# Zhehui-Huang/quad-swarm-rl

Hardware: AMD Instinct MI355X
Metric: env-steps/s (drones x envs x sim_steps) (higher is better)
Workload: dtype f32

## Files before the change

__graft_entry__.py:

```python
import os
import subprocess
import sys

REPO = os.path.dirname(os.path.abspath(__file__))
if REPO not in sys.path:
    sys.path.insert(0, REPO)


def build():
    from quad_swarm_rl_amd import native
    native.build(force=True, verbose=True)
    assert os.path.exists(native.LIB_PATH)
    from quad_swarm_rl_amd import policy
    policy.build(force=True, verbose=True)
    assert os.path.exists(policy.ENC_LIB_PATH)
    subprocess.check_call(["make", "-C", os.path.join(REPO, "oracle"), "-s", "-B"])
    import quad_swarm_rl_amd
    from quad_swarm_rl_amd import config, env
    import ctypes
    lib = ctypes.CDLL(native.LIB_PATH)
    for sym in native.EXPORTED_SYMBOLS + native.EXCHANGE_SYMBOLS:
        getattr(lib, sym)
    paths = prebuild_spec_cache()
    print(f"build ok: {native.LIB_PATH} + {len(paths)} config-specialised code objects in spec_cache/")
# ... 32 lines not shown
        import test_object_identity_gpu as toi
        for name in toi.POISON_CASES:
            for team in (0, 1):
                kw = dict(thp.CASES[name], num_envs=7, **toi.POISON_OVERRIDES.get(name, {}))
                prec = "f32" if team and kw["num_agents"] > 8 else "f64"
                jobs.append((kw, prec, team))
                jobs += [(kw, prec, team, {"QS_SPEC_EXTRA_FLAGS": f"-DQS_POISON_IDLE={m}"}) for m in (1, 2)]
        for name in toi.SCHED_SINGLE:
            jobs += [(dict(thp.CASES[name], num_envs=7), "f32", 0), (dict(thp.CASES[name], num_envs=7), "f32", 0, {"QS_SPEC_SINGLE_FLAGS": "-mllvm -amdgpu-use-amdgpu-trackers"})]
        for name in ("c2_n8_dw", "c3_n8_obst", "c4_n32_svs"):
            jobs += [(dict(thp.CASES[name], num_envs=7), "f32", 1), (dict(thp.CASES[name], num_envs=7), "f32", 1, {"QS_SPEC_TEAM_FLAGS": ""})]
        for name in toi.RESPONSE_CASES:
            for prec in ("f64", "f32"):
                if prec == "f64" and thp.CASES[name]["num_agents"] > 8:
                    continue
                jobs += [(dict(thp.CASES[name], num_envs=7), prec, 1), (dict(thp.CASES[name], num_envs=7), prec, 1, {"QS_SPEC_EXTRA_FLAGS": "-DQS_SERIAL_PAIR_RESPONSES"})]
        for name in toi.SELECT_CASES:
            jobs += [(dict(thp.CASES[name], num_envs=7), "f32", 0)] + [(dict(thp.CASES[name], num_envs=7), "f32", 0, {"QS_SPEC_EXTRA_FLAGS": f})
                                                                       for f in ("-DQS_EXACT_NBR_SELECT", "-DQS_NBR_TRUNC_BITS=16")]
        for name in toi.STASH_CASES:
            jobs += [(dict(thp.CASES[name], num_envs=7), "f32", 1), (dict(thp.CASES[name], num_envs=7), "f32", 1, {"QS_SPEC_EXTRA_FLAGS": "-DQS_SN_STASH=0"})]
        for name in toi.REDO_CASES:
            jobs += [(dict(thp.CASES[name], num_envs=7), "f32", 1), (dict(thp.CASES[name], num_envs=7), "f32", 1, {"QS_SPEC_EXTRA_FLAGS": "-DQS_REDO_ROWS=0"})]
        import xchg_worker as xw
        jobs += [(dict(xw.KW, num_envs=8, write_rew_info=False), "f32"), (dict(xw.KW, num_envs=4, episode_sums=True), "f32"),
                 (dict(xw.REPLAY_KW, num_envs=8, write_rew_info=False, episode_sums=True), "f32")]
        import test_pilot_gpu as tpg
        jobs.append((dict(tpg.LOOP_KW, num_envs=1024), "f32"))
        import test_replay_gpu as trg
        jobs += trg.spec_jobs()
    except Exception as exc:
        print("spec prebuild: parity cases skipped:", exc)
    finally:
        sys.path.pop(0)
    if with_audit:
        jobs += _audit_jobs()
    return jobs


def _audit_jobs():
    import base64
    import ctypes
    import json
    from quad_swarm_rl_amd import config as qcfg
    path = os.path.join(REPO, "tests", "spec_audit.json")
    if not os.path.exists(path):
# ... 89 lines not shown
```

quad-swarm-rl_amd/csrc/qs_state_rows.h:

```cpp
#pragma once
#include "qs_state_blk.h"
#include "qs_xchg_dev.h"

template <typename real> struct Ptrs {
    StateBlk blk;
    real *pos, *vel, *rot, *omega, *rot_damp, *cmds_damp, *ou, *goal;
    uint32_t *flags;
    uint64_t *pair_mask, *new_pair_mask;
    real *obs, *reward, *rew_info;
    uint8_t *done;
    int32_t *obst_hit_idx;
    uint64_t *unique_col, *obst_new, *room_new;
    int32_t *counters, *tick;
    uint32_t *step_ctr;
    real *obst_pos;
    real *dist_ring, *dist_sums;
    real *ep_stats;
    int32_t *ep_counters;
    real *scen_real;
    int32_t *scen_int;
    uint32_t *error_flag;
    uint64_t *scen_omap;
    int32_t *scenario_id;
    int32_t *ep_scenario;
// ... 68 lines not shown
            for (int k = 0; k < K; ++k) st(src[k], k);
            return;
        }
        constexpr int D = K * (int)sizeof(T) / 4;
        uint32_t w[D];
#pragma unroll
        for (int k = 0; k < K; ++k) {
            if constexpr (sizeof(T) == 8) { const uint64_t u = __builtin_bit_cast(uint64_t, src[k]); w[2 * k] = (uint32_t)u;
                w[2 * k + 1] = (uint32_t)(u >> 32); }
            else w[k] = __builtin_bit_cast(uint32_t, src[k]);
        }
        st_dwords<D>(w, 0);
    }
};
#define QS_BUF_RSRC(p) __builtin_amdgcn_make_buffer_rsrc((void *)(p).blk.base, 0, (p).blk.bytes, 0x00020000)
#define QS_BLK blockIdx.x
#if defined(QS_SPEC_TEAM)
#define QS_LM(p) (QS_SPEC_TEAM == 8)
#else
#define QS_LM(p) ((p).blk.lane_major != 0)
#endif
#define QS_ROW(TYPE, name, rs, p, T, g) const BufRow<TYPE> b_##name = {rs, (uint32_t)(QS_BLK * (p).blk.block_bytes + (p).blk.name), (uint32_t)((QS_LM(p) ? 1 : 64) * sizeof(TYPE)), \
                                                                       (uint32_t)((threadIdx.x & 63) * ((QS_LM(p) ? blkc::name : 1) * sizeof(TYPE))), QS_LM(p)}
#define QS_ROWF(TYPE, name, rs, p, T, g) const BufRow<TYPE> b_##name = {rs, (p).blk.name, (uint32_t)((T) * sizeof(TYPE)), (uint32_t)((g) * sizeof(TYPE)), false}
```

quad-swarm-rl_amd/csrc/qs_step_team.inc:

```
#undef e_state_or_e
#if QS_MULTI
#define e_state_or_e e_state
#else
#define e_state_or_e e
#endif
#ifndef QS_GATED
#define QS_GATED 0
#endif
#ifdef QS_SPEC
#if QS_MULTI && QS_GATED
extern "C" __global__ void __launch_bounds__(64 * QS_TW) qs_spec_gated(QS_KARGS, int QS_EPB_ARG, int ksteps) {
#elif QS_MULTI
extern "C" __global__ void __launch_bounds__(64 * QS_TW) qs_spec_rollout(QS_KARGS, int QS_EPB_ARG, int ksteps) {
#else
extern "C" __global__ void __launch_bounds__(64 * QS_TW) qs_spec_step(QS_KARGS, int QS_EPB_ARG) {
    const int t = 0;
#endif
#else
template <typename real>
#if QS_MULTI && QS_GATED && QS_SCEN_FULL
__global__ void __launch_bounds__(64 * QS_TW) qs_gated_team_full(QS_KARGS, int QS_EPB_ARG, int ksteps) {
#elif QS_MULTI && QS_GATED
__global__ void __launch_bounds__(64 * QS_TW) qs_gated_team(QS_KARGS, int QS_EPB_ARG, int ksteps) {
#elif QS_MULTI && QS_SCEN_FULL
__global__ void __launch_bounds__(64 * QS_TW) qs_rollout_team_full(QS_KARGS, int QS_EPB_ARG, int ksteps) {
#elif QS_MULTI
__global__ void __launch_bounds__(64 * QS_TW) qs_rollout_team(QS_KARGS, int QS_EPB_ARG, int ksteps) {
#elif QS_SCEN_FULL
__global__ void __launch_bounds__(64 * QS_TW) qs_step_team_full(QS_KARGS, int QS_EPB_ARG) {
    const int t = 0;
// ... 35 lines not shown
#endif
#endif
#ifndef QS_REDO_ROWS
#ifdef QS_SPEC
#define QS_REDO_ROWS 1
#else
#define QS_REDO_ROWS 0
#endif
#endif

    QS_POISON_LDS(L.total, 64 * QS_TW);
    const int wv = __builtin_amdgcn_readfirstlane((int)(threadIdx.x >> 6));
    const int tid = threadIdx.x & 63, le = tid / N, i = tid - le * N, e = blockIdx.x * epb + le, base = le * N;
    const bool active = (le < epb) && (e < E);
    const int g = active ? e * N + i : 0, ee = active ? e : 0;
    const uint64_t nmask = (N >= 64) ? ~0ull : ((1ull << N) - 1);
    real *myobs = s_obs + tid * c.obs_dim;
    const __amdgpu_buffer_rsrc_t rs = QS_BUF_RSRC(p);
    QS_ROW(real, pos, rs, p, T, g); QS_ROW(real, vel, rs, p, T, g); QS_ROW(real, rot, rs, p, T, g); QS_ROW(real, omega, rs, p, T, g);
    QS_ROW(real, rot_damp, rs, p, T, g); QS_ROW(real, cmds_damp, rs, p, T, g); QS_ROW(real, ou, rs, p, T, g);
    QS_ROW(real, goal, rs, p, T, g);
    QS_ROW(real, ring, rs, p, T, g); QS_ROW(real, sums, rs, p, T, g); QS_ROW(uint32_t, flags, rs, p, T, g);
    QS_ROW(uint64_t, pair, rs, p, T, g);

    QS_STAMP(0);
    QS_STAMPW(0);
    QS_STAMP_WG(0);
    Drone<real> d;
    real goal[3], act[4], ring[4], sums[3];
    int32_t cnt[QS_CNT_COUNT];
    uint64_t prev_pair = 0;
    int tick_before = 0, svs_period = 0;
#if QS_SCEN_FULL && defined(QS_SPEC_N)
    ScenRegs<real> sreg;
#endif
    uint32_t step_no = 0;
    uint32_t step_raw = 0;
    if (wv <= 1 || (QS_SN_STASH && !QS_MULTI && wv == 2)) step_raw = p.step_ctr[ee];
    if (wv == 0) {
        if (b_pos.wide) {
            b_pos.template ldv<3>(d.pos); b_vel.template ldv<3>(d.vel); b_omega.template ldv<3>(d.omega); b_goal.template ldv<3>(goal);
            b_sums.template ldv<3>(sums);
            b_rot.template ldv<9>(d.rot);
            b_rot_damp.template ldv<4>(d.rot_damp); b_cmds_damp.template ldv<4>(d.cmds_damp); b_ou.template ldv<4>(d.ou);
            b_ring.template ldv<4>(ring);
        } else {
#pragma unroll
            for (int q = 0; q < 3; ++q) { d.pos[q] = b_pos.ld(q); d.vel[q] = b_vel.ld(q); d.omega[q] = b_omega.ld(q);
                goal[q] = b_goal.ld(q); sums[q] = b_sums.ld(q); }
#pragma unroll
            for (int q = 0; q < 9; ++q) d.rot[q] = b_rot.ld(q);
#pragma unroll
            for (int q = 0; q < 4; ++q) { d.rot_damp[q] = b_rot_damp.ld(q); d.cmds_damp[q] = b_cmds_damp.ld(q); d.ou[q] = b_ou.ld(q);
                ring[q] = b_ring.ld(q); }
        }
        d.flags = b_flags.ld();
        prev_pair = b_pair.ld();
        QS_POISON_DRONE(d); QS_POISON_ARR(goal, 3, 16); QS_POISON_ARR(sums, 3, 16); QS_POISON_ARR(ring, 4, 16); QS_POISON_U64(prev_pair);
        tick_before = p.tick[ee];
        svs_period = (c.scenario == QS_SCENARIO_SWARM_VS_SWARM) ? p.scen_int[ee] : 0;
        if (active && i == 0) {
// ... 9 lines not shown
#endif
        asm volatile("" : "+v"(step_raw));
        step_no = step_raw + 1;
    } else if (wv == 1 || (QS_SN_STASH && !QS_MULTI && wv == 2)) {
        step_no = step_raw + 1;
    }
    if (wv == W - 1 && c.use_obstacles && active) {
        for (int k = i; k < M_; k += N) {
            s_obst[(le * 2 + 0) * M_ + k] = p.obst_pos[(size_t)e * M_ + k];
            s_obst[(le * 2 + 1) * M_ + k] = p.obst_pos[(size_t)E * M_ + (size_t)e * M_ + k];
        }
    }
#if QS_SCEN_FULL
    real *s_sr = (real *)(smem + L.off_sr) + le * SR_COUNT;
    int *s_si = (int *)(smem + L.off_si) + le * SI_COUNT;
#endif
    constexpr int WL = 2;
    const bool logw = (wv == WL) && active;
    real rsum[QS_SUM_COUNT];
    if (logw && c.episode_sums) {
#pragma unroll
        for (int q = 0; q < QS_SUM_COUNT; ++q) rsum[q] = p.run_sums[q * T + g];
    }
#if !QS_MULTI
    unsigned long long xq_seq = 0, xq_ack = ~0ull;
    if constexpr (sizeof(real) == 4) {
        if (p.xchg != nullptr) {
            xq_seq = p.xchg->loc->push_seq;
            if (wv == 0 && tid < p.xchg->world) xq_ack = qsx::ld_sys(&p.xchg->mine->ack[tid]);
        }
    }
#endif
    uint64_t out_curr_pair = 0;
    bool nan_any = false;
#if QS_MULTI
    const int g_state = g, e_state = e;
#if QS_GATED
    qsx::Gate *const G = (qsx::Gate *)p.xchg;
    const unsigned long long gseq0 = (unsigned long long)(uintptr_t)actions;
    bool gate_dead = false;
    unsigned long long *s_pre_seq = (unsigned long long *)s_ri;
    unsigned int *s_actpre = (unsigned int *)((char *)s_ri + 16);
    unsigned long long pf_flag = 0, pf_flag_next = 0;
    if (threadIdx.x == 0) *s_pre_seq = 0;
#endif
    for (int t = 0; t < ksteps; ++t) {
    int g = g_state, e = e_state;
// ... 670 lines not shown
        int nenv = E - first_env; nenv = nenv < epb ? nenv : epb;
        const int total = nenv * N * D;
        real *dst = p.obs + (size_t)first_env * N * D;
#if QS_GATED
        {
            if ((total & 3) == 0 && ((((size_t)first_env * N * D) * sizeof(real)) & 15) == 0 && sizeof(real) == 4) {
                const qsx::u32x4_t *src4 = (const qsx::u32x4_t *)s_obs;
                for (int idx = threadIdx.x; idx < total / 4; idx += 64 * W) qsx::st16_sc1((float *)dst + 4 * idx, src4[idx]);
            } else if constexpr (sizeof(real) == 4) {
                for (int idx = threadIdx.x; idx < total; idx += 64 * W) qsx::st4_sc1(dst + idx, __float_as_uint((float)s_obs[idx]));
            } else {
                for (int idx = threadIdx.x; idx < total; idx += 64 * W) qsx::st8_sc1(dst + idx,
                    (unsigned long long)__double_as_longlong((double)s_obs[idx]));
            }
        }
#else
        if ((total & 3) == 0 && ((((size_t)first_env * N * D) * sizeof(real)) & 15) == 0 && sizeof(real) == 4) {
            const qs_f32x4 *src4 = (const qs_f32x4 *)s_obs;
            for (int idx = threadIdx.x; idx < total / 4; idx += 64 * W) obs_st4((float *)dst + 4 * idx, src4[idx]);
        } else {
            for (int idx = threadIdx.x; idx < total; idx += 64 * W) obs_st1<real>(dst + idx, s_obs[idx]);
        }
#endif
#if !QS_MULTI
        if constexpr (sizeof(real) == 4) {
            if (p.xchg != nullptr) {
                const qsx::XchgDev &X = *p.xchg;
                const unsigned long long seq = xq_seq + 1;
                const int slot = (int)(seq & 1);
                if (wv == 0) {
                    bool ok = true;
                    if (tid < X.world && seq > 2 && xq_ack < seq - 2) ok = qsx::poll_ge(&X.mine->ack[tid], seq - 2, X.timeout_ticks);
                    if (__any(!ok) && tid == 0) atomicOr(&X.loc->status, (unsigned int)QS_XCHG_ERR_ACK_TIMEOUT);
                }
                __syncthreads();
                const size_t row0 = (size_t)first_env * N * D, wsz = X.wire == QS_WIRE_BF16 ? 2 : 4;
                const size_t off = X.wire == QS_WIRE_Q8 ? (size_t)slot * (size_t)X.slot_bytes + ((size_t)X.rank * (size_t)(X.n / D) + (size_t)first_env * N) * (size_t)X.q8.row_words * 4
                                                        : (size_t)slot * (size_t)X.slot_bytes + ((size_t)X.rank * (size_t)X.n + row0) * wsz;
                const float *src = (const float *)s_obs;
                const bool vec = ((total & 7) == 0) && ((off & 15) == 0);
#ifndef QS_NO_Q8_FUSED
                if (X.wire == QS_WIRE_Q8) {
                    const int q0 = c.self_dim, q1 = c.self_dim + 6 * K, w16 = (D - 6 * K + 1) >> 1;
                    const float s0 = X.q8.s0, s1 = X.q8.s1, s2 = X.q8.s2, s3 = X.q8.s3, s4 = X.q8.s4, s5 = X.q8.s5;
                    const int rw = w16 + ((6 * K + 3) >> 2), words = nenv * N * rw;
                    unsigned int *s_wire = (unsigned int *)s_ri;
                    if ((off & 15) == 0 && (words & 3) == 0 && words * 4 <= (int)(sizeof(real) * (QS_RI_COUNT + 1) * B)) {
// ... 103 lines not shown
                qsx::st8_sc1(p.room_new + e, out_room); }
        }
        if (wv == 1) {
            if (pf_hold_issue) {
#pragma unroll
                for (int q = 0; q < (int)sizeof(real); ++q) s_actpre[tid * (int)sizeof(real) + q] = pf_hold[q];
            }
            if (tid == 0) *s_pre_seq = pf_hold_issue ? gseq0 + (unsigned long long)t + 2 : 0ull;
            pf_flag = pf_flag_next;
        }
        asm volatile("s_waitcnt vmcnt(0)" ::: "memory");
        QS_TEAM_BARRIER();
        if (threadIdx.x == 0) qsx::st_agent(&G->done_flag[blockIdx.x], gseq0 + (unsigned long long)t + 1);
    }
#else
    if (wv == 0 && active) {
        {
            QS_ROWF(uint64_t, newpair, rs, p, T, g); QS_ROWF(int32_t, ohit, rs, p, T, g); QS_ROWF(real, reward, rs, p, T, g);
            QS_ROWF(uint8_t, done, rs, p, T, g);
            b_newpair.st(out_new_pair);
            if (c.use_obstacles) b_ohit.st(out_obst_idx);
            b_reward.st(rew); b_done.st(done ? 1 : 0);
        }
        if (i == 0) { p.unique_col[e] = out_unique; p.obst_new[e] = out_obst_new; p.room_new[e] = out_room; }
    }
#endif
    nan_any |= nan_rew;
    prev_pair = out_curr_pair;
    tick_before = out_tick;
    step_no += 1;
#if QS_MULTI
    }
#endif

    if (logw && c.episode_sums) {
#if QS_MULTI
        const int g = g_state;
#endif
#pragma unroll
        for (int q = 0; q < QS_SUM_COUNT; ++q) p.run_sums[q * T + g] = rsum[q];
    }
    if (wv == 0) {
#if QS_SCEN_FULL
        QS_WAVE_SYNC();
        if (active) scen_lds_store<real>(p, L, smem, E, e_state_or_e, le, i, N);
#endif
        if (active) {
// ... 9 lines not shown
            QS_ROW(real, ring, rs, p, Ts, g); QS_ROW(real, sums, rs, p, Ts, g); QS_ROW(uint32_t, flags, rs, p, Ts, g);
            QS_ROW(uint64_t, pair, rs, p, Ts, g);
            if (b_pos.wide) {
                b_vel.template stv<3>(d.vel); b_omega.template stv<3>(d.omega);
                b_pos.template stv<3>(d.pos); b_rot.template stv<9>(d.rot);
                b_rot_damp.template stv<4>(d.rot_damp); b_cmds_damp.template stv<4>(d.cmds_damp); b_ou.template stv<4>(d.ou);
            } else {
#pragma unroll
                for (int q = 0; q < 3; ++q) { b_vel.st(d.vel[q], q); b_omega.st(d.omega[q], q); }
#pragma unroll
                for (int q = 0; q < 3; ++q) b_pos.st(d.pos[q], q);
#pragma unroll
                for (int q = 0; q < 9; ++q) b_rot.st(d.rot[q], q);
#pragma unroll
                for (int q = 0; q < 4; ++q) { b_rot_damp.st(d.rot_damp[q], q); b_cmds_damp.st(d.cmds_damp[q], q); b_ou.st(d.ou[q], q); }
            }
            b_flags.st(d.flags);
            b_goal.template stv<3>(goal);
            b_sums.template stv<3>(sums);
            b_ring.template stv<4>(ring);
            b_pair.st(out_curr_pair);
            if (nan_any) atomicOr(p.error_flag, 1u);
            if (i == 0) {
#pragma unroll
                for (int q = 0; q < QS_CNT_COUNT; ++q) p.counters[q * E + e] = cnt[q];
                p.tick[e] = tick_before;
                p.step_ctr[e] = step_no - 1;
            }
        }
    }
    QS_STAMP(13);
    QS_STAMP_WG(1);
}
```

quad-swarm-rl_amd/csrc/qs_step_team_modes.inc:

```
#define QS_MULTI 0
#include "qs_step_team.inc"
#undef QS_MULTI
#define QS_MULTI 1
#include "qs_step_team.inc"
#undef QS_GATED
#define QS_GATED 1
#include "qs_step_team.inc"
#undef QS_GATED
#undef QS_MULTI
```

quad-swarm-rl_amd/csrc/quadswarm_hip.hip:

```cpp
#include <hip/hip_runtime.h>

#include <cctype>
#include <cmath>
#include <cstdio>
#include <cstdlib>
#include <cstring>
#include <dlfcn.h>
#include <sys/stat.h>
#include <unistd.h>

#include <string>
#include <vector>

#include "qs_codeobj_check.h"
#include "qs_kernels.h"
#include "qs_replay_kernels.h"
#include "qs_env_plan.h"
#include "qs_pilot.h"
#include "qs_summary.h"

using namespace qs_check;

extern "C" int qs_tape_lds_bytes(const qs_config *cfg, int obs_dim, int full, int real_size);
extern "C" int qs_tape_launch(int which, const qs_config *cfg, int obs_dim, int full, int real_size, const void *consts,
    const void *ptrs, const void *actions, void *stream);
static thread_local std::string g_last_error;
static int fail(int code, const std::string &msg) { g_last_error = msg; return code; }
#define HIP_TRY(expr) do { hipError_t _e = (expr); if (_e != hipSuccess) return fail(QS_ERR_HIP, std::string(#expr) + ": " + hipGetErrorString(_e)); } while (0)

struct qs_handle {
    qs_config cfg;
    int device = 0;
    int real_size = 4;
    int obs_dim = 0, epb = 1, blocks = 0;
    LdsLayout lds;
    bool full = false;
    int cus = 256;
    int team = 0;
    struct SnapArray { char *base; size_t elem, comps, comp_stride, per_env; int kind; size_t group, group_stride; };
    std::vector<SnapArray> snap_arrays;
    size_t snap_bytes = 0;
    char *snap_pool = nullptr;
    int32_t snap_slots = 0;
    hipModule_t spec_mod = nullptr;
    hipFunction_t spec_step = nullptr, spec_rollout = nullptr, spec_reset = nullptr, spec_gated = nullptr;
    std::string spec_note;
    Consts<float> kf;
    Consts<double> kd;
    Ptrs<float> pf;
    std::vector<void *> allocs;
    qs_buffers bufs;
    void *d_actions = nullptr;
    void *obs_target = nullptr;
    double *d_state_buf = nullptr;
    int32_t *d_tick_io = nullptr;
    hipStream_t cap_stream = nullptr;
    hipGraphExec_t graph_exec = nullptr;
    const void *graph_actions = nullptr;
    int32_t graph_k = 0;
    uint8_t *h_mask = nullptr;
    bool replay_on = false;
    bool replay_stepped = false;
    ReplayParams rp;
    double *d_tape = nullptr;
    int32_t *d_tape_pos = nullptr;
    int64_t tape_len = 0;
    qsx::Gate *d_gate = nullptr;
    qsx::Gate gate_host = {};
// ... 187 lines not shown
        typedef BlkOff<real> BO;
        if ((int)block_bytes != qs_block_bytes((int)R) || block_bytes != BO::bytes || o_pos != BO::pos || o_vel != BO::vel ||
            o_rot != BO::rot || o_omega != BO::omega || o_rd != BO::rot_damp || o_cd != BO::cmds_damp || o_ou != BO::ou ||
            o_goal != BO::goal || o_ring != BO::ring || o_sums != BO::sums || o_flags != BO::flags || o_pair != BO::pair)
            return fail(QS_ERR_INVALID, "state block layout out of step with BlkOff / qs_block_bytes()");
        size_t off = NBLK * block_bytes;
        auto carve = [&](size_t bytes) { size_t o = off; off = (off + bytes + 255) & ~(size_t)255; return o; };
        const size_t o_newpair = carve(T * 8), o_reward = carve(T * R), o_done = carve(T), o_ohit = carve(T * 4);
        if (off >= ((size_t)1 << 32))
            return fail(QS_ERR_UNSUPPORTED, "per-drone state exceeds the 4 GiB a buffer resource addresses: use fewer envs per handle");
        char *blk = nullptr;
        if ((rc = dalloc(h, &blk, off)) != QS_OK) return rc;
        p.blk = {blk, (uint32_t)off, (uint32_t)block_bytes, (uint32_t)EPB, (uint32_t)o_pos, (uint32_t)o_vel, (uint32_t)o_rot,
                 (uint32_t)o_omega, (uint32_t)o_rd, (uint32_t)o_cd, (uint32_t)o_ou, (uint32_t)o_goal, (uint32_t)o_ring, (uint32_t)o_sums,
                 (uint32_t)o_flags, (uint32_t)o_pair, (uint32_t)o_newpair, (uint32_t)o_reward, (uint32_t)o_done, (uint32_t)o_ohit,
                 (uint32_t)(h->team == 8 ? 1 : 0)};
        p.pos = (real *)(blk + o_pos); p.vel = (real *)(blk + o_vel); p.rot = (real *)(blk + o_rot); p.omega = (real *)(blk + o_omega);
        p.rot_damp = (real *)(blk + o_rd); p.cmds_damp = (real *)(blk + o_cd); p.ou = (real *)(blk + o_ou); p.goal = (real *)(blk + o_goal);
        p.dist_ring = (real *)(blk + o_ring); p.dist_sums = (real *)(blk + o_sums); p.flags = (uint32_t *)(blk + o_flags);
        p.pair_mask = (uint64_t *)(blk + o_pair); p.new_pair_mask = (uint64_t *)(blk + o_newpair); p.reward = (real *)(blk + o_reward);
        p.done = (uint8_t *)(blk + o_done); p.obst_hit_idx = (int32_t *)(blk + o_ohit);
    }
    DA(obs, T * D); DA(rew_info, QS_RI_COUNT * T);
    DA(unique_col, E); DA(obst_new, E); DA(room_new, E); DA(counters, QS_CNT_COUNT * E); DA(tick, E); DA(step_ctr, E);
    DA(obst_pos, 2 * E * (M_ ? M_ : 1)); DA(ep_stats, QS_EPS_COUNT * T); DA(ep_counters, QS_CNT_COUNT * E);
    DA(run_sums, QS_SUM_COUNT * T); DA(ep_sums, QS_SUM_COUNT * T);
    DA(obst_count, E); DA(obst_size_env, E); DA(obst_density_env, E);
    {
        int32_t *dc = nullptr; real *dd = nullptr, *ds = nullptr;
        if ((rc = dalloc(h, &dc, QS_MAX_DR_CHOICES)) != QS_OK || (rc = dalloc(h, &dd, QS_MAX_DR_CHOICES)) != QS_OK
            || (rc = dalloc(h, &ds, QS_MAX_DR_CHOICES)) != QS_OK) return rc;
        real hd[QS_MAX_DR_CHOICES], hs[QS_MAX_DR_CHOICES];
        for (int q = 0; q < QS_MAX_DR_CHOICES; ++q) { hd[q] = (real)c.dr_density[q]; hs[q] = (real)c.dr_size[q]; }
        HIP_TRY(hipMemcpy(dc, c.dr_obst_count, sizeof c.dr_obst_count, hipMemcpyHostToDevice));
        HIP_TRY(hipMemcpy(dd, hd, sizeof hd, hipMemcpyHostToDevice));
        HIP_TRY(hipMemcpy(ds, hs, sizeof hs, hipMemcpyHostToDevice));
        p.dr_count = dc; p.dr_density = dd; p.dr_size = ds;
    }
    {
        std::vector<int32_t> cnt(E, c.num_obstacles);
        std::vector<real> sz(E, (real)c.obst_size), dn(E, (real)c.obst_density);
        HIP_TRY(hipMemcpy(p.obst_count, cnt.data(), E * sizeof(int32_t), hipMemcpyHostToDevice));
        HIP_TRY(hipMemcpy(p.obst_size_env, sz.data(), E * sizeof(real), hipMemcpyHostToDevice));
        HIP_TRY(hipMemcpy(p.obst_density_env, dn.data(), E * sizeof(real), hipMemcpyHostToDevice));
    }
    DA(scen_real, SR_COUNT * E); DA(scen_int, SI_COUNT * E); DA(scen_omap, 4 * E); DA(scenario_id, E); DA(ep_scenario, E);
    {
// ... 41 lines not shown
    SNAP_T(run_sums, QS_SUM_COUNT); sa.back().kind = 2;
    sa.push_back({(char *)p.obs, sizeof(real), 1, T * D, N * D, 1, 0, 0});
    SNAP_E(unique_col, 1); SNAP_E(obst_new, 1); SNAP_E(room_new, 1); SNAP_E(counters, QS_CNT_COUNT); SNAP_E(tick, 1);
    SNAP_E(scen_real, SR_COUNT); SNAP_E(scen_int, SI_COUNT); SNAP_E(scen_omap, 4); SNAP_E(scenario_id, 1);
    SNAP_E(obst_count, 1); SNAP_E(obst_size_env, 1); SNAP_E(obst_density_env, 1);
    sa.push_back({(char *)p.obst_pos, sizeof(real), 2, E * (M_ ? M_ : 1), (M_ ? M_ : 1), 0, 0, 0});
#undef SNAP_T
#undef SNAP_B
#undef SNAP_E
    h->snap_bytes = 0;
    for (const auto &a : sa) h->snap_bytes += (a.elem * a.comps * a.per_env + 15) & ~(size_t)15;
    return QS_OK;
}

struct KernelEntry { const void *fn; int threads; };
enum { MODE_STEP = 0, MODE_ROLLOUT, MODE_GATED, MODE_COUNT };
#define QS_BOTH(KERNEL, THREADS) {{(const void *)KERNEL<float>, THREADS}, {(const void *)KERNEL<double>, THREADS}}
static const KernelEntry kStepKernels[2][2][MODE_COUNT][2] = {
    {{QS_BOTH(qs_step_kernel, QS_WAVE), QS_BOTH(qs_rollout_kernel, QS_WAVE), {}},
     {QS_BOTH(qs_step_kernel_full, QS_WAVE), QS_BOTH(qs_rollout_kernel_full, QS_WAVE), {}}},
    {{QS_BOTH(qs_step_team, QS_TEAM_THREADS), QS_BOTH(qs_rollout_team, QS_TEAM_THREADS), QS_BOTH(qs_gated_team, QS_TEAM_THREADS)},
     {QS_BOTH(qs_step_team_full, QS_TEAM_THREADS), QS_BOTH(qs_rollout_team_full, QS_TEAM_THREADS), QS_BOTH(qs_gated_team_full, QS_TEAM_THREADS)}}};
#undef QS_BOTH
static const KernelEntry kResetKernels[2][2] = {
    {{(const void *)qs_reset_kernel<float, false>, QS_WAVE}, {(const void *)qs_reset_kernel<double, false>, QS_WAVE}},
    {{(const void *)qs_reset_kernel<float, true>, QS_WAVE}, {(const void *)qs_reset_kernel<double, true>, QS_WAVE}}};
static bool raise_lds_limit(const KernelEntry *k, size_t count, int bytes) {
    for (; count--; ++k)
        if (k->fn && hipFuncSetAttribute(k->fn, hipFuncAttributeMaxDynamicSharedMemorySize, bytes) != hipSuccess) return false;
    return true;
}
static const char *const kGatedNeedsTeam = "resident-state stepping lives in the team kernels (batches up to ~8 waves per CU, see qs_kernel_flavor): larger batches are bandwidth-bound, not launch-bound";

extern "C" {

int qs_version(void) { return QS_VERSION; }
size_t qs_sizeof_config(void) { return sizeof(qs_config); }
const char *qs_last_error(void) { return g_last_error.c_str(); }

int qs_obs_dim(const qs_config *c) { return qs_self_dim(c->obs_repr) + 6 * c->num_neighbors + (c->use_obstacles ? 9 : 0); }

int qs_default_config(qs_config *c, int32_t num_envs, int32_t num_agents) {
    memset(c, 0, sizeof *c);
    c->num_envs = num_envs; c->num_agents = num_agents; c->precision = QS_PRECISION_F32; c->seed = 0;
    c->mass = 0.028000000000000008; c->arm = 0.04596194077712559;
    c->inertia[0] = 1.3669232142857143e-05; c->inertia[1] = 1.4356732142857143e-05; c->inertia[2] = 2.656158333333334e-05;
    const double pc[4][3] = {{-0.0325, -0.0325, 0}, {-0.0325, 0.0325, 0}, {0.0325, 0.0325, 0}, {0.0325, -0.0325, 0}};
    const double ccw[4] = {-1, 1, -1, 1};
    for (int m = 0; m < 4; ++m) {
        for (int q = 0; q < 3; ++q) c->prop_cross[m][q] = pc[m][q];
        c->prop_ccw[m] = ccw[m];
        c->thrust_max[m] = 9.81 * c->mass * 1.9 / 4.0;
        c->torque_max[m] = 0.006 * c->thrust_max[m];
    }
// ... 44 lines not shown
        h->team = team_default(h->blocks, cus, cfg->num_agents) ? QS_TEAM_WAVES : 0;
        h->cus = cus;
        if (team_ch == '0') h->team = 0;
        else if (team_ch == '1' || team_ch == '4' || team_ch == '8') h->team = QS_TEAM_WAVES;
    }
    {
        const char *ev = getenv("QS_SPEC");
        const std::string mode = (ev && ev[0]) ? ev : "jit";
        const int spec_team = h->team ? (team_ch == '4' ? 4 : (team_ch == '8' ? 8 : spec_team_waves(cfg->num_agents))) : 0;
        const LdsLayout sl = handle_layout(cfg, spec_team, true);
        const bool require = mode == "require";
        if (mode == "off" || mode == "0") h->spec_note = "QS_SPEC=off";
        else if (sl.total > 64 * 1024) h->spec_note = "LDS layout above the 64 KiB a module-loaded kernel gets";
        else {
            const std::string path = spec_ensure(cfg, spec_team, mode == "jit" || require);
            if (!path.empty()) {
                if (hipModuleLoad(&h->spec_mod, path.c_str()) == hipSuccess &&
                    hipModuleGetFunction(&h->spec_step, h->spec_mod, "qs_spec_step") == hipSuccess &&
                    hipModuleGetFunction(&h->spec_rollout, h->spec_mod, "qs_spec_rollout") == hipSuccess &&
                    hipModuleGetFunction(&h->spec_reset, h->spec_mod, "qs_spec_reset") == hipSuccess) {
                    h->team = spec_team;
                    if (spec_team > 0 && hipModuleGetFunction(&h->spec_gated, h->spec_mod, "qs_spec_gated") != hipSuccess) {
                        (void)hipGetLastError(); h->spec_gated = nullptr; }
                } else {
                    (void)hipGetLastError();
                    if (h->spec_mod) { (void)hipModuleUnload(h->spec_mod); h->spec_mod = nullptr; }
                    h->spec_step = h->spec_rollout = h->spec_reset = h->spec_gated = nullptr;
                    h->spec_note = "cannot load " + path;
                }
            } else {
                h->spec_note = g_last_error;
            }
        }
        if (!h->spec_step && mode != "off" && mode != "0") {
            if (require && sl.total <= 64 * 1024) { const std::string why = h->spec_note; delete h;
                return fail(QS_ERR_UNSUPPORTED, "QS_SPEC=require: no config-specialised kernels: " + why); }
            fprintf(stderr, "quadswarm_hip: WARNING: running the GENERIC step kernels (%s)\n", h->spec_note.c_str());
        }
    }
    h->lds = handle_layout(cfg, h->team, h->spec_step != nullptr);
    h->full = scenario_is_full(cfg->scenario);
    rc = (h->real_size == 8) ? create_typed<double>(h) : create_typed<float>(h);
    if (rc == QS_OK) {
        if (hipMalloc((void **)&h->d_state_buf, sizeof(double) * QS_MAX_AGENTS * QS_STATE_STRIDE) != hipSuccess ||
            hipMalloc((void **)&h->d_tick_io, sizeof(int32_t)) != hipSuccess ||
            hipHostMalloc((void **)&h->h_mask, (size_t)cfg->num_envs) != hipSuccess)
            rc = fail(QS_ERR_HIP, "allocation failed");
    }
    if (rc != QS_OK) { qs_destroy(h); return rc; }
    if (h->lds.total > 64 * 1024 && !(raise_lds_limit(&kStepKernels[0][0][0][0], sizeof kStepKernels / sizeof(KernelEntry), h->lds.total) &&
                                      raise_lds_limit(&kResetKernels[0][0], sizeof kResetKernels / sizeof(KernelEntry), h->lds.total))) {
        qs_destroy(h);
        return fail(QS_ERR_HIP, "cannot raise dynamic LDS limit");
    }
    *out = h;
    return QS_OK;
}

int qs_is_specialized(qs_handle *h) { return (h && h->spec_step) ? 1 : 0; }
int qs_spec_status(qs_handle *h, char *why_out, int cap) {
    if (!h) return fail(QS_ERR_INVALID, "null handle");
    if (why_out && cap > 0) { snprintf(why_out, (size_t)cap, "%s", h->spec_note.c_str()); }
    return h->spec_step ? 1 : 0;
}
int qs_kernel_flavor(qs_handle *h) {
    return h ? ((h->spec_step ? 1 : 0) | (h->team ? 2 : 0) | (h->full ? 4 : 0) | ((h->team ? h->team : 1) << 8)) : 0;
}

int qs_destroy(qs_handle *h) {
    if (!h) return QS_OK;
    (void)hipSetDevice(h->device);
    (void)hipDeviceSynchronize();
    if (h->spec_mod) { (void)hipModuleUnload(h->spec_mod); h->spec_mod = nullptr; }
    if (h->snap_pool) (void)hipFree(h->snap_pool);
    for (void *q : h->allocs) (void)hipFree(q);
    if (h->d_state_buf) (void)hipFree(h->d_state_buf);
    if (h->d_tick_io) (void)hipFree(h->d_tick_io);
    if (h->h_mask) (void)hipHostFree(h->h_mask);
    if (h->d_tape) (void)hipFree(h->d_tape);
    if (h->d_tape_pos) (void)hipFree(h->d_tape_pos);
    if (h->d_gate) (void)hipFree(h->d_gate);
    if (h->gate_stream) (void)hipStreamDestroy(h->gate_stream);
    if (h->gate_ev_in) (void)hipEventDestroy(h->gate_ev_in);
    if (h->gate_ev_out) (void)hipEventDestroy(h->gate_ev_out);
    for (auto &ev : h->events) { (void)hipEventDestroy(ev.first); (void)hipEventDestroy(ev.second); }
    if (h->graph_exec) (void)hipGraphExecDestroy(h->graph_exec);
    if (h->cap_stream) (void)hipStreamDestroy(h->cap_stream);
    free(h->pilot);
    if (h->summary) (void)hipFree(h->summary);
// ... 26 lines not shown
            hipEvent_t a, b;
            HIP_TRY(hipEventCreate(&a)); HIP_TRY(hipEventCreate(&b));
            h->events.emplace_back(a, b);
        }
        e0 = h->events[h->events_used].first; e1 = h->events[h->events_used].second;
        ++h->events_used;
        HIP_TRY(hipEventRecord(e0, s));
    }
    if (h->d_tape) {
        const size_t stride = (size_t)h->cfg.num_envs * h->cfg.num_agents * 4 * (size_t)h->real_size;
        for (int t = 0; t < ksteps; ++t) {
            hipError_t e = (hipError_t)qs_tape_launch(1, &h->cfg, h->obs_dim, h->full ? 1 : 0, h->real_size,
                                                     h->real_size == 8 ? (const void *)&h->kd : (const void *)&h->kf, &h->pf,
                                                     (const char *)actions + stride * t, s);
            if (e != hipSuccess) return fail(QS_ERR_HIP, std::string("tape step kernel: ") + hipGetErrorString(e));
        }
        if (h->profiling) HIP_TRY(hipEventRecord(e1, s));
        return QS_OK;
    }
    Ptrs<float> pf = h->pf;
    if (h->obs_target) pf.obs = (float *)h->obs_target;
    if (pf.xchg != nullptr && ksteps > 1)
        return fail(QS_ERR_UNSUPPORTED, "multi-step launches do not exchange observation rows: qs_set_obs_exchange is active");
    if (gated) pf.xchg = (const qsx::XchgDev *)h->d_gate;
    void *args[] = {h->real_size == 8 ? (void *)&h->kd : (void *)&h->kf, &pf, (void *)&actions, &h->lds, &h->epb, &ksteps};
    if (h->spec_step) {
        if (gated && !h->spec_gated)
            return fail(QS_ERR_UNSUPPORTED, "the specialised code object of this handle has no resident-state kernel");
        HIP_TRY(hipModuleLaunchKernel(gated ? h->spec_gated : (ksteps == 1 ? h->spec_step : h->spec_rollout), h->blocks, 1, 1,
                                      h->team ? QS_WAVE * h->team : QS_WAVE, 1, 1, h->lds.total, s, args, nullptr));
    } else {
        const KernelEntry &k = kStepKernels[h->team != 0][h->full][gated ? MODE_GATED : (ksteps == 1 ? MODE_STEP : MODE_ROLLOUT)][h->real_size == 8];
        if (!k.fn) return fail(QS_ERR_UNSUPPORTED, kGatedNeedsTeam);
        HIP_TRY(hipLaunchKernel(k.fn, dim3(h->blocks), dim3(k.threads), args, h->lds.total, s));
    }
    if (h->profiling) HIP_TRY(hipEventRecord(e1, s));
    return QS_OK;
}

static int launch_replay(qs_handle *h, hipStream_t s) {
    hipLaunchKernelGGL(qs_replay_kernel, dim3(h->cfg.num_envs), dim3(QS_WAVE), 0, s, h->rp);
    HIP_TRY(hipGetLastError());
    return QS_OK;
}

#include "qs_gate.inc"

extern "C" {

int qs_reset(qs_handle *h, const uint8_t *env_mask_host, void *stream) {
    if (!h) return fail(QS_ERR_INVALID, "null handle");
    HIP_TRY(hipSetDevice(h->device));
    if (int jr = gate_join_stream(h, (hipStream_t)stream)) return jr;
    hipStream_t s = (hipStream_t)stream;
    const int E = h->cfg.num_envs;
    for (int e = 0; e < E; ++e) h->h_mask[e] = env_mask_host ? (env_mask_host[e] ? 1 : 0) : 1;
// ... 67 lines not shown
            h->pf.done, h->pf.ep_sums, h->pf.ep_stats, h->pf.ep_counters, h->pf.ep_scenario, h->pf.scenario_id,
            h->replay_on ? h->rp.ep_saved : nullptr, h->replay_on ? h->rp.last_steps : nullptr, &h->summary};
    return QS_OK;
}

int qs_set_obs_target(qs_handle *h, void *obs_dev) {
    if (!h) return fail(QS_ERR_INVALID, "null handle");
    if (obs_dev && h->replay_on)
        return fail(QS_ERR_UNSUPPORTED, "qs_set_obs_target: the device-side replay wrapper restores observations into qs_buffers.obs");
    if (obs_dev && h->d_tape) return fail(QS_ERR_UNSUPPORTED, "qs_set_obs_target: not available while a noise tape is set");
    h->obs_target = obs_dev;
    return QS_OK;
}

extern "C" void *qs_xchg_fused_desc(struct qs_xchg *x, int32_t blocks, int32_t auto_ack, int64_t *n_out);
extern "C" const char *qs_xchg_last_error(void);
extern "C" int qs_xchg_row_layout_is(struct qs_xchg *x, int32_t cols, int32_t q0, int32_t q1);
int qs_set_obs_exchange(qs_handle *h, struct qs_xchg *xchg, int32_t auto_ack) {
    if (!h) return fail(QS_ERR_INVALID, "null handle");
    if (!xchg) { h->pf.xchg = nullptr; return QS_OK; }
    if (!h->team || h->real_size != 4)
        return fail(QS_ERR_UNSUPPORTED, "qs_set_obs_exchange: the fused exchange lives in the float32 team kernels (small batches); use qs_xchg_push for this handle");
    if (h->d_tape) return fail(QS_ERR_UNSUPPORTED, "qs_set_obs_exchange: not available while a noise tape is set");
    HIP_TRY(hipSetDevice(h->device));
    int64_t n = 0;
    void *desc = qs_xchg_fused_desc(xchg, h->blocks, auto_ack, &n);
    if (!desc) return fail(QS_ERR_INVALID, std::string("qs_set_obs_exchange: ") + qs_xchg_last_error());
    if (n != (int64_t)h->cfg.num_envs * h->cfg.num_agents * h->obs_dim)
        return fail(QS_ERR_INVALID, "qs_set_obs_exchange: the endpoint's rows * cols must be E*N * obs_dim");
    {
        const int self_dim = qs_self_dim(h->cfg.obs_repr);
        if (!qs_xchg_row_layout_is(xchg, h->obs_dim, self_dim, self_dim + 6 * h->cfg.num_neighbors))
            return fail(QS_ERR_INVALID, "qs_set_obs_exchange: the endpoint's row layout is not this configuration's (QS_WIRE_Q8: q0 = self columns, q1 = q0 + 6 * visible neighbours)");
    }
    h->pf.xchg = (const qsx::XchgDev *)desc;
    return QS_OK;
}

int qs_set_reward_coeffs(qs_handle *h, const double *coeffs) {
    if (!h || !coeffs) return fail(QS_ERR_INVALID, "null argument");
    HIP_TRY(hipSetDevice(h->device));
    HIP_TRY(hipDeviceSynchronize());
    for (int q = 0; q < QS_REW_COUNT; ++q) h->cfg.rew_coeff[q] = coeffs[q];
    fill_consts<float>(h->cfg, h->kf);
    fill_consts<double>(h->cfg, h->kd);
    return h->real_size == 8 ? upload_reward_coeffs(h->kd, h->pf.rew_rt) : upload_reward_coeffs(h->kf, h->pf.rew_rt);
// ... 17 lines not shown
```

quad-swarm-rl_amd/native.py:

```python
import ctypes as C
import os
import re
import sys
import subprocess

import numpy as np

from . import abi
from . import config as qcfg
from .abi import QS_OK, QS_ERR_NAN_REWARD, QsBuffers, GateInfo, PilotParams, WireQ8

HERE = os.path.dirname(os.path.abspath(__file__))
CSRC = os.path.join(HERE, "csrc")
LIB_PATH = os.environ.get("QS_LIB", os.path.join(CSRC, "libquadswarm_hip.so"))
UNITS = [os.path.join(CSRC, n) for n in ("quadswarm_hip.hip", "qs_tape_kernels.hip", "qs_exchange.hip", "qs_codeobj_check.cpp", "qs_pilot.hip", "qs_episode_summary.hip")]
UNIT_FLAGS = {"qs_tape_kernels.hip": ["-ffp-contract=off"], "qs_episode_summary.hip": ["-ffp-contract=off"], "qs_pilot.hip": ["-fno-fast-math", "-fhip-fp32-correctly-rounded-divide-sqrt"]}
CHECK_TOOL = os.path.join(CSRC, "qs_spec_check")


def include_closure(units):
    seen, todo = [], list(units)
    while todo:
        path = todo.pop()
        if path not in seen:
# ... 326 lines not shown
        _check(lib().qs_set_tape_pos(self._h, a.ctypes.data_as(C.POINTER(C.c_int32))))

    @property
    def specialized(self):
        return bool(lib().qs_is_specialized(self._h))

    @property
    def spec_note(self):
        buf = C.create_string_buffer(1024)
        lib().qs_spec_status(self._h, buf, len(buf))
        return buf.value.decode()

    @property
    def team(self):
        return bool(lib().qs_kernel_flavor(self._h) & 2)

    @property
    def waves_per_workgroup(self):
        return (lib().qs_kernel_flavor(self._h) >> 8) & 0xff

    @property
    def kernel_name(self):
        fl = lib().qs_kernel_flavor(self._h)
        if fl & 1:
            return "qs_spec_step"
        real = "float" if self.real_size == 4 else "double"
        return ("qs_step_team" if fl & 2 else "qs_step_kernel") + ("_full" if fl & 4 else "") + f"<{real}>"

    def kernel_time(self):
        ms, n = C.c_double(0), C.c_int64(0)
        _check(lib().qs_get_kernel_time(self._h, C.byref(ms), C.byref(n)))
        return ms.value, n.value

    def _dtype(self, kind):
        return {"real": self.np_real, "u1": np.uint8, "u4": np.uint32, "i4": np.int32, "u8": np.uint64}[kind]

    def ptr(self, name):
        return getattr(self.bufs, name)

    BLOCKED = frozenset(("pos", "vel", "omega", "rot", "thrust_rot_damp", "thrust_cmds_damp", "ou_state", "goal", "flags", "col_pair_mask"))

    def to_host(self, name):
        shape, kind = self._shapes[name]
        out = np.empty(shape, dtype=self._dtype(kind))
        if name in self.BLOCKED:
            _check(lib().qs_state_array_copy(self._h, out.ctypes.data_as(C.c_void_p), C.c_void_p(self.ptr(name)), out.dtype.itemsize,
                                             shape[0] if len(shape) == 2 else 1, 0))
        else:
            _check(lib().qs_memcpy_d2h(self._h, out.ctypes.data_as(C.c_void_p), C.c_void_p(self.ptr(name)), out.nbytes))
        return out
# ... 32 lines not shown
```

Baseline: 2.344 billion.

## Split exchange-epilogue step kernel out and pack per-env rows into one buffer

```diff
diff --git a/__graft_entry__.py b/__graft_entry__.py
--- a/__graft_entry__.py
+++ b/__graft_entry__.py
@@ -78,6 +78,10 @@
             jobs += [(dict(thp.CASES[name], num_envs=7), "f32", 1), (dict(thp.CASES[name], num_envs=7), "f32", 1, {"QS_SPEC_EXTRA_FLAGS": "-DQS_SN_STASH=0"})]
         for name in toi.REDO_CASES:
             jobs += [(dict(thp.CASES[name], num_envs=7), "f32", 1), (dict(thp.CASES[name], num_envs=7), "f32", 1, {"QS_SPEC_EXTRA_FLAGS": "-DQS_REDO_ROWS=0"})]
+        import test_step_flavours_gpu as tsf
+        for name in tsf.FLAVOUR_CASES:
+            jobs += [(dict(thp.CASES[name], num_envs=7), "f32", 1)] + [(dict(thp.CASES[name], num_envs=7), "f32", 1, {"QS_SPEC_EXTRA_FLAGS": f})
+                                                                       for f in tsf.FLAVOUR_FLAGS]
         import xchg_worker as xw
         jobs += [(dict(xw.KW, num_envs=8, write_rew_info=False), "f32"), (dict(xw.KW, num_envs=4, episode_sums=True), "f32"),
                  (dict(xw.REPLAY_KW, num_envs=8, write_rew_info=False, episode_sums=True), "f32")]
diff --git a/quad-swarm-rl_amd/csrc/qs_state_rows.h b/quad-swarm-rl_amd/csrc/qs_state_rows.h
--- a/quad-swarm-rl_amd/csrc/qs_state_rows.h
+++ b/quad-swarm-rl_amd/csrc/qs_state_rows.h
@@ -114,4 +114,13 @@
 #endif
 #define QS_ROW(TYPE, name, rs, p, T, g) const BufRow<TYPE> b_##name = {rs, (uint32_t)(QS_BLK * (p).blk.block_bytes + (p).blk.name), (uint32_t)((QS_LM(p) ? 1 : 64) * sizeof(TYPE)), \
                                                                        (uint32_t)((threadIdx.x & 63) * ((QS_LM(p) ? blkc::name : 1) * sizeof(TYPE))), QS_LM(p)}
+#define QS_ENVROW_unique 0
+#define QS_ENVROW_obst_new 2
+#define QS_ENVROW_room_new 4
+#define QS_ENVROW_counters 6
+#define QS_ENVROW_tick (6 + QS_CNT_COUNT)
+#define QS_ENVROW_step_ctr (7 + QS_CNT_COUNT)
+#define QS_ENVROW_COUNT (8 + QS_CNT_COUNT)
+#define QS_ENV_RSRC(p, E) __builtin_amdgcn_make_buffer_rsrc((void *)(p).unique_col, 0, (uint32_t)(QS_ENVROW_COUNT * 4) * (uint32_t)(E), 0x00020000)
+#define QS_ROWE(TYPE, name, rs, E, e) const BufRow<TYPE> b_##name = {rs, (uint32_t)(QS_ENVROW_##name * 4) * (uint32_t)(E), 4u * (uint32_t)(E), (uint32_t)((e) * sizeof(TYPE)), false}
 #define QS_ROWF(TYPE, name, rs, p, T, g) const BufRow<TYPE> b_##name = {rs, (p).blk.name, (uint32_t)((T) * sizeof(TYPE)), (uint32_t)((g) * sizeof(TYPE)), false}
diff --git a/quad-swarm-rl_amd/csrc/qs_step_team.inc b/quad-swarm-rl_amd/csrc/qs_step_team.inc
--- a/quad-swarm-rl_amd/csrc/qs_step_team.inc
+++ b/quad-swarm-rl_amd/csrc/qs_step_team.inc
@@ -6,6 +6,9 @@
 #endif
 #ifndef QS_GATED
 #define QS_GATED 0
+#endif
+#ifndef QS_XCHG
+#error "QS_XCHG (0 / 1: the one-step body with the fused exchange epilogue) comes from qs_step_team_modes.inc"
 #endif
 #ifdef QS_SPEC
 #if QS_MULTI && QS_GATED
@@ -87,6 +90,15 @@
     QS_ROW(real, goal, rs, p, T, g);
     QS_ROW(real, ring, rs, p, T, g); QS_ROW(real, sums, rs, p, T, g); QS_ROW(uint32_t, flags, rs, p, T, g);
     QS_ROW(uint64_t, pair, rs, p, T, g);
+#ifndef QS_ENV_ROWS_FLAT
+#define QS_ENV_ROWS_FLAT 1
+#endif
+#undef QS_ENV_ROWS
+#define QS_ENV_ROWS (QS_ENV_ROWS_FLAT && !QS_MULTI)
+#if QS_ENV_ROWS
+    const __amdgpu_buffer_rsrc_t rs_env = QS_ENV_RSRC(p, E);
+    QS_ROWE(uint32_t, step_ctr, rs_env, E, ee);
+#endif
 
     QS_STAMP(0);
     QS_STAMPW(0);
@@ -101,7 +113,13 @@
 #endif
     uint32_t step_no = 0;
     uint32_t step_raw = 0;
-    if (wv <= 1 || (QS_SN_STASH && !QS_MULTI && wv == 2)) step_raw = p.step_ctr[ee];
+    if (wv <= 1 || (QS_SN_STASH && !QS_MULTI && wv == 2)) {
+#if QS_ENV_ROWS
+        step_raw = b_step_ctr.ld();
+#else
+        step_raw = p.step_ctr[ee];
+#endif
+    }
     if (wv == 0) {
         if (b_pos.wide) {
             b_pos.template ldv<3>(d.pos); b_vel.template ldv<3>(d.vel); b_omega.template ldv<3>(d.omega); b_goal.template ldv<3>(goal);
@@ -157,7 +175,7 @@
 #pragma unroll
         for (int q = 0; q < QS_SUM_COUNT; ++q) rsum[q] = p.run_sums[q * T + g];
     }
-#if !QS_MULTI
+#if !QS_MULTI && QS_XCHG
     unsigned long long xq_seq = 0, xq_ack = ~0ull;
     if constexpr (sizeof(real) == 4) {
         if (p.xchg != nullptr) {
@@ -874,7 +892,7 @@
             for (int idx = threadIdx.x; idx < total; idx += 64 * W) obs_st1<real>(dst + idx, s_obs[idx]);
         }
 #endif
-#if !QS_MULTI
+#if !QS_MULTI && QS_XCHG
         if constexpr (sizeof(real) == 4) {
             if (p.xchg != nullptr) {
                 const qsx::XchgDev &X = *p.xchg;
@@ -1024,7 +1042,9 @@
             if (c.use_obstacles) b_ohit.st(out_obst_idx);
             b_reward.st(rew); b_done.st(done ? 1 : 0);
         }
+#if !QS_ENV_ROWS
         if (i == 0) { p.unique_col[e] = out_unique; p.obst_new[e] = out_obst_new; p.room_new[e] = out_room; }
+#endif
     }
 #endif
     nan_any |= nan_rew;
@@ -1080,10 +1100,22 @@
             b_pair.st(out_curr_pair);
             if (nan_any) atomicOr(p.error_flag, 1u);
             if (i == 0) {
+#if QS_ENV_ROWS
+                uint32_t Es = (uint32_t)__builtin_amdgcn_readfirstlane((int)E);
+                asm volatile("" : "+s"(Es));
+                QS_ROWE(uint64_t, unique, rs_env, Es, e); QS_ROWE(uint64_t, obst_new, rs_env, Es, e); QS_ROWE(uint64_t, room_new, rs_env, Es, e);
+                QS_ROWE(int32_t, counters, rs_env, Es, e); QS_ROWE(int32_t, tick, rs_env, Es, e); QS_ROWE(uint32_t, step_ctr, rs_env, Es, e);
+                b_unique.st(out_unique); b_obst_new.st(out_obst_new); b_room_new.st(out_room);
+#pragma unroll
+                for (int q = 0; q < QS_CNT_COUNT; ++q) b_counters.st(cnt[q], q);
+                b_tick.st(tick_before);
+                b_step_ctr.st(step_no - 1);
+#else
 #pragma unroll
                 for (int q = 0; q < QS_CNT_COUNT; ++q) p.counters[q * E + e] = cnt[q];
                 p.tick[e] = tick_before;
                 p.step_ctr[e] = step_no - 1;
+#endif
             }
         }
     }
diff --git a/quad-swarm-rl_amd/csrc/qs_step_team_modes.inc b/quad-swarm-rl_amd/csrc/qs_step_team_modes.inc
--- a/quad-swarm-rl_amd/csrc/qs_step_team_modes.inc
+++ b/quad-swarm-rl_amd/csrc/qs_step_team_modes.inc
@@ -1,5 +1,23 @@
+#ifndef QS_XCHG_INLINE
+#define QS_XCHG_INLINE 0
+#endif
+#define QS_TEAM_BODY "qs_step_team.inc"
 #define QS_MULTI 0
+#define QS_XCHG QS_XCHG_INLINE
 #include "qs_step_team.inc"
+#undef QS_XCHG
+#if !QS_XCHG_INLINE && !(defined(QS_SPEC) && QS_SPEC_PRECISION == 8)
+#define QS_XCHG 1
+#define qs_spec_step qs_spec_step_x
+#define qs_step_team qs_step_team_x
+#define qs_step_team_full qs_step_team_full_x
+#include QS_TEAM_BODY
+#undef qs_spec_step
+#undef qs_step_team
+#undef qs_step_team_full
+#undef QS_XCHG
+#endif
+#define QS_XCHG 0
 #undef QS_MULTI
 #define QS_MULTI 1
 #include "qs_step_team.inc"
@@ -8,3 +26,5 @@
 #include "qs_step_team.inc"
 #undef QS_GATED
 #undef QS_MULTI
+#undef QS_XCHG
+#undef QS_TEAM_BODY
diff --git a/quad-swarm-rl_amd/csrc/quadswarm_hip.hip b/quad-swarm-rl_amd/csrc/quadswarm_hip.hip
--- a/quad-swarm-rl_amd/csrc/quadswarm_hip.hip
+++ b/quad-swarm-rl_amd/csrc/quadswarm_hip.hip
@@ -43,7 +43,7 @@
     char *snap_pool = nullptr;
     int32_t snap_slots = 0;
     hipModule_t spec_mod = nullptr;
-    hipFunction_t spec_step = nullptr, spec_rollout = nullptr, spec_reset = nullptr, spec_gated = nullptr;
+    hipFunction_t spec_step = nullptr, spec_rollout = nullptr, spec_reset = nullptr, spec_gated = nullptr, spec_step_x = nullptr;
     std::string spec_note;
     Consts<float> kf;
     Consts<double> kd;
@@ -277,7 +277,13 @@
         p.done = (uint8_t *)(blk + o_done); p.obst_hit_idx = (int32_t *)(blk + o_ohit);
     }
     DA(obs, T * D); DA(rew_info, QS_RI_COUNT * T);
-    DA(unique_col, E); DA(obst_new, E); DA(room_new, E); DA(counters, QS_CNT_COUNT * E); DA(tick, E); DA(step_ctr, E);
+    {
+        uint32_t *rows = nullptr;
+        if ((rc = dalloc(h, &rows, (size_t)QS_ENVROW_COUNT * E)) != QS_OK) return rc;
+        p.unique_col = (uint64_t *)(rows + QS_ENVROW_unique * E); p.obst_new = (uint64_t *)(rows + QS_ENVROW_obst_new * E);
+        p.room_new = (uint64_t *)(rows + QS_ENVROW_room_new * E); p.counters = (int32_t *)(rows + QS_ENVROW_counters * E);
+        p.tick = (int32_t *)(rows + QS_ENVROW_tick * E); p.step_ctr = rows + QS_ENVROW_step_ctr * E;
+    }
     DA(obst_pos, 2 * E * (M_ ? M_ : 1)); DA(ep_stats, QS_EPS_COUNT * T); DA(ep_counters, QS_CNT_COUNT * E);
     DA(run_sums, QS_SUM_COUNT * T); DA(ep_sums, QS_SUM_COUNT * T);
     DA(obst_count, E); DA(obst_size_env, E); DA(obst_density_env, E);
@@ -365,6 +371,12 @@
     {{QS_BOTH(qs_step_team, QS_TEAM_THREADS), QS_BOTH(qs_rollout_team, QS_TEAM_THREADS), QS_BOTH(qs_gated_team, QS_TEAM_THREADS)},
      {QS_BOTH(qs_step_team_full, QS_TEAM_THREADS), QS_BOTH(qs_rollout_team_full, QS_TEAM_THREADS), QS_BOTH(qs_gated_team_full, QS_TEAM_THREADS)}}};
 #undef QS_BOTH
+#if QS_XCHG_INLINE
+static const KernelEntry kStepXchgKernels[2] = {{nullptr, 0}, {nullptr, 0}};
+#else
+static const KernelEntry kStepXchgKernels[2] = {
+    {(const void *)qs_step_team_x<float>, QS_TEAM_THREADS}, {(const void *)qs_step_team_full_x<float>, QS_TEAM_THREADS}};
+#endif
 static const KernelEntry kResetKernels[2][2] = {
     {{(const void *)qs_reset_kernel<float, false>, QS_WAVE}, {(const void *)qs_reset_kernel<double, false>, QS_WAVE}},
     {{(const void *)qs_reset_kernel<float, true>, QS_WAVE}, {(const void *)qs_reset_kernel<double, true>, QS_WAVE}}};
@@ -373,6 +385,7 @@
         if (k->fn && hipFuncSetAttribute(k->fn, hipFuncAttributeMaxDynamicSharedMemorySize, bytes) != hipSuccess) return false;
     return true;
 }
+static const char *const kNoXchgKernel = "qs_set_obs_exchange: this handle's kernels have no one-step kernel with the exchange epilogue (qs_spec_step_x / qs_step_team_x: float32 team kernels, not built with -DQS_XCHG_INLINE=1)";
 static const char *const kGatedNeedsTeam = "resident-state stepping lives in the team kernels (batches up to ~8 waves per CU, see qs_kernel_flavor): larger batches are bandwidth-bound, not launch-bound";
 
 extern "C" {
@@ -463,10 +476,12 @@
                     h->team = spec_team;
                     if (spec_team > 0 && hipModuleGetFunction(&h->spec_gated, h->spec_mod, "qs_spec_gated") != hipSuccess) {
                         (void)hipGetLastError(); h->spec_gated = nullptr; }
+                    if (spec_team > 0 && hipModuleGetFunction(&h->spec_step_x, h->spec_mod, "qs_spec_step_x") != hipSuccess) {
+                        (void)hipGetLastError(); h->spec_step_x = nullptr; }
                 } else {
                     (void)hipGetLastError();
                     if (h->spec_mod) { (void)hipModuleUnload(h->spec_mod); h->spec_mod = nullptr; }
-                    h->spec_step = h->spec_rollout = h->spec_reset = h->spec_gated = nullptr;
+                    h->spec_step = h->spec_rollout = h->spec_reset = h->spec_gated = h->spec_step_x = nullptr;
                     h->spec_note = "cannot load " + path;
                 }
             } else {
@@ -490,6 +505,7 @@
     }
     if (rc != QS_OK) { qs_destroy(h); return rc; }
     if (h->lds.total > 64 * 1024 && !(raise_lds_limit(&kStepKernels[0][0][0][0], sizeof kStepKernels / sizeof(KernelEntry), h->lds.total) &&
+                                      raise_lds_limit(&kStepXchgKernels[0], sizeof kStepXchgKernels / sizeof(KernelEntry), h->lds.total) &&
                                       raise_lds_limit(&kResetKernels[0][0], sizeof kResetKernels / sizeof(KernelEntry), h->lds.total))) {
         qs_destroy(h);
         return fail(QS_ERR_HIP, "cannot raise dynamic LDS limit");
@@ -505,7 +521,7 @@
     return h->spec_step ? 1 : 0;
 }
 int qs_kernel_flavor(qs_handle *h) {
-    return h ? ((h->spec_step ? 1 : 0) | (h->team ? 2 : 0) | (h->full ? 4 : 0) | ((h->team ? h->team : 1) << 8)) : 0;
+    return h ? ((h->spec_step ? 1 : 0) | (h->team ? 2 : 0) | (h->full ? 4 : 0) | (h->pf.xchg ? 8 : 0) | ((h->team ? h->team : 1) << 8)) : 0;
 }
 
 int qs_destroy(qs_handle *h) {
@@ -578,16 +594,19 @@
     if (h->obs_target) pf.obs = (float *)h->obs_target;
     if (pf.xchg != nullptr && ksteps > 1)
         return fail(QS_ERR_UNSUPPORTED, "multi-step launches do not exchange observation rows: qs_set_obs_exchange is active");
+    const bool with_xchg = pf.xchg != nullptr && !gated;
     if (gated) pf.xchg = (const qsx::XchgDev *)h->d_gate;
     void *args[] = {h->real_size == 8 ? (void *)&h->kd : (void *)&h->kf, &pf, (void *)&actions, &h->lds, &h->epb, &ksteps};
     if (h->spec_step) {
         if (gated && !h->spec_gated)
             return fail(QS_ERR_UNSUPPORTED, "the specialised code object of this handle has no resident-state kernel");
-        HIP_TRY(hipModuleLaunchKernel(gated ? h->spec_gated : (ksteps == 1 ? h->spec_step : h->spec_rollout), h->blocks, 1, 1,
+        if (with_xchg && !h->spec_step_x) return fail(QS_ERR_UNSUPPORTED, kNoXchgKernel);
+        HIP_TRY(hipModuleLaunchKernel(gated ? h->spec_gated : (ksteps == 1 ? (with_xchg ? h->spec_step_x : h->spec_step) : h->spec_rollout), h->blocks, 1, 1,
                                       h->team ? QS_WAVE * h->team : QS_WAVE, 1, 1, h->lds.total, s, args, nullptr));
     } else {
-        const KernelEntry &k = kStepKernels[h->team != 0][h->full][gated ? MODE_GATED : (ksteps == 1 ? MODE_STEP : MODE_ROLLOUT)][h->real_size == 8];
-        if (!k.fn) return fail(QS_ERR_UNSUPPORTED, kGatedNeedsTeam);
+        const KernelEntry &k = with_xchg ? kStepXchgKernels[h->full]
+                                         : kStepKernels[h->team != 0][h->full][gated ? MODE_GATED : (ksteps == 1 ? MODE_STEP : MODE_ROLLOUT)][h->real_size == 8];
+        if (!k.fn) return fail(QS_ERR_UNSUPPORTED, with_xchg ? kNoXchgKernel : kGatedNeedsTeam);
         HIP_TRY(hipLaunchKernel(k.fn, dim3(h->blocks), dim3(k.threads), args, h->lds.total, s));
     }
     if (h->profiling) HIP_TRY(hipEventRecord(e1, s));
@@ -701,6 +720,7 @@
     if (!h->team || h->real_size != 4)
         return fail(QS_ERR_UNSUPPORTED, "qs_set_obs_exchange: the fused exchange lives in the float32 team kernels (small batches); use qs_xchg_push for this handle");
     if (h->d_tape) return fail(QS_ERR_UNSUPPORTED, "qs_set_obs_exchange: not available while a noise tape is set");
+    if (h->spec_step ? !h->spec_step_x : !kStepXchgKernels[h->full].fn) return fail(QS_ERR_UNSUPPORTED, kNoXchgKernel);
     HIP_TRY(hipSetDevice(h->device));
     int64_t n = 0;
     void *desc = qs_xchg_fused_desc(xchg, h->blocks, auto_ack, &n);
diff --git a/quad-swarm-rl_amd/native.py b/quad-swarm-rl_amd/native.py
--- a/quad-swarm-rl_amd/native.py
+++ b/quad-swarm-rl_amd/native.py
@@ -372,10 +372,11 @@
     @property
     def kernel_name(self):
         fl = lib().qs_kernel_flavor(self._h)
+        x = "_x" if fl & 8 else ""
         if fl & 1:
-            return "qs_spec_step"
+            return "qs_spec_step" + x
         real = "float" if self.real_size == 4 else "double"
-        return ("qs_step_team" if fl & 2 else "qs_step_kernel") + ("_full" if fl & 4 else "") + f"<{real}>"
+        return ("qs_step_team" if fl & 2 else "qs_step_kernel") + ("_full" if fl & 4 else "") + x + f"<{real}>"
 
     def kernel_time(self):
         ms, n = C.c_double(0), C.c_int64(0)
```

After: 2.417 billion, median of 6. 1.03x the previous value.
